# ChenWu98/cycle-diffusion

Measured on AMD Instinct MI355X. Metric: images/sec, SD-v1.4 512px CycleDiffusion 100+100 steps, 1/2/4/8 MI355X, higher is better.
Workload: dtype fp16; 1 GPU; C2: Stable-Diffusion-v1.4-shaped U-Net + KL-f8 VAE, 512x512, custom_steps=99 white_box_steps=100 eta=0.1 skip 0, 1 trial, encoder scale 1, decoder CFG 3; batch_per_gpu=4, global_batch=4, parallelism=dp1, steps_per_launch_set=5, launch_set_cap=16, launch_sets_in_flight_per_gpu=1, images_in_flight_per_gpu=20, distributed=single process, weights=synthetic(seed=0)

## Files before the change

cycle-diffusion_amd/_ffi.py:

```python
import ctypes as C
import os

import numpy as np

_HERE = os.path.dirname(os.path.abspath(__file__))
LIB_PATH = os.path.join(_HERE, "lib", "libcyclediff.so")

CD_NET_UNET_OPENAI, CD_NET_UNET_HO, CD_NET_VAE_KL, CD_NET_CLIP_TEXT, CD_NET_BERT_XTR = 1, 2, 3, 4, 5
CD_NET_OCLIP_TEXT, CD_NET_OCLIP_VISION, CD_NET_INCEPTION_FID, CD_NET_LPIPS = 6, 7, 8, 9
CD_SCHED_DDIM, CD_SCHED_DDPM = 0, 1
CD_PREC_16, CD_PREC_F32, CD_PREC_F32X3 = 0, 1, 2
CD_MASK_QSAMPLE, CD_MASK_ENCODER = 0, 1
MASK_SOURCES = {"q_sample": CD_MASK_QSAMPLE, "encoder": CD_MASK_ENCODER}
ACT_NONE, ACT_SILU, ACT_GELU, ACT_GEGLU, ACT_QGELU, ACT_RELU = 0, 1, 2, 3, 4, 5


class NetDesc(C.Structure):
    _fields_ = [
        ("kind", C.c_int), ("image_size", C.c_int), ("in_channels", C.c_int), ("out_channels", C.c_int),
        ("model_channels", C.c_int), ("num_res_blocks", C.c_int),
        ("n_mult", C.c_int), ("channel_mult", C.c_int * 8),
        ("n_attn", C.c_int), ("attn", C.c_int * 8),
        ("num_heads", C.c_int), ("num_head_channels", C.c_int),
        ("use_spatial_transformer", C.c_int), ("context_dim", C.c_int), ("transformer_depth", C.c_int),
# ... 55 lines not shown
                              _U64, _VP],
    "cd_cycle_translate_masked": [_VP, _I, _I, _VP, _VP, _VP, _F, _VP, _VP, _F, _VP, _I, _I, _I, _I, _VP, _VP, _VP, _U64, _I,
                                  _VP, _VP, _I, _I, _VP, _VP, _U64, _VP, _VP],
    "cd_cycle_translate_ctrl": [_VP, _I, _I, _VP, _VP, _VP, _F, _VP, _VP, _F, _VP, _I, _I, _I, _I, _VP, _VP, _VP, _U64, _I,
                                _VP, _VP, _I, _I, _VP, _VP, _U64, _VP, _VP, _VP, _I, _I, _VP, _VP],
    "cd_cycle_translate_blend": [_VP, _I, _I, _VP, _VP, _VP, _F, _VP, _VP, _F, _VP, _I, _I, _I, _I, _VP, _VP, _VP, _U64, _I,
                                 _VP, _VP, _VP, _I, _I, _VP, _VP, _I, _I, _I, _F, _I, _VP, _VP, _VP, _VP],
    "cd_cycle_translate_sega": [_VP, _I, _I, _VP, _VP, _VP, _F, _VP, _VP, _F, _VP, _I, _I, _I, _I, _VP, _VP, _VP, _U64, _I,
                                _VP, _VP, _I, _I, _VP, _VP, _U64, _VP, _VP, _VP, _I, _I, _VP, _VP, _I, _F, _F, _VP, _VP, _VP,
                                _VP, _VP],
    "cd_ilvr_decode": [_VP, _I, _I, _VP, _I, _I, _I, _I, _VP, _VP, _U64, _VP, _I, _I, _I, _VP, _VP, _U64, _VP],
    "cd_automask": [_VP, _I, _VP, _VP, _VP, _I, _I, _I, _I, _F, _F, _VP, _U64, _I, _F, _F, _I, _VP, _VP],
    "cd_word_maps": [_VP, _I, _VP, _VP, _I, _I, _VP, _I, _I, _I, _I, _F, _F, _VP, _U64, _I, _I, _I, _VP, C.POINTER(_I)],
    "cd_pix_refine": [_VP, _I, _I, _VP, _I, _I, _VP, _VP, _U64],
    "cd_op_pack_conv_weight": [_VP, _VP, _I, _I, _I, _I, _I, C.POINTER(_VP), C.POINTER(_I), C.POINTER(_I)],
    "cd_op_free": [_VP, _VP],
    "cd_op_conv2d": [_VP, _VP, _I, _VP, _I, _I, _I, _I, _VP, _I, _I, _I, _I, _I, _I, _I, _VP, _VP, _VP, _I, _I, _VP],
    "cd_op_conv2d_16": [_VP, _VP, _I, _VP, _I, _I, _I, _I, _VP, _I, _I, _I, _I, _I, _I, _I, _VP, _VP, _VP, _I, _I, _VP,
                        _VP],
    "cd_op_last_gemm_config": [_VP] + [C.POINTER(_I)] * 5,
    "cd_op_up_phase_reorder": [_VP, _VP, _I, _I, _I, _I, _VP],
    "cd_op_groupnorm": [_VP, _VP, _I, _I, _I, _I, _I, _F, _VP, _VP, _VP, _I, _VP],
    "cd_op_groupnorm_ex": [_VP, _VP, _I, _I, _VP, _I, _I, _I, _I, _I, _F, _VP, _VP, _VP, _I, _I, _VP, _VP, _I, _VP],
    "cd_op_pack_conv_weight_prec": [_VP, _VP, _I, _I, _I, _I, _I, C.POINTER(_VP)],
    "cd_op_conv2d_prec": [_VP, _VP, _I, _I, _VP, _I, _I, _I, _I, _I, _VP, _I, _I, _I, _I, _I, _I, _I, _VP, _VP, _I, _VP, _I, _I,
                          _I, _I, _I, _I, _F, _VP, _VP],
    "cd_op_attention_prec": [_VP, _VP, _VP, _VP, _I, _I, _I, _I, _I, _I, _I, _I, _F, _I, _VP, _I, _I, _VP],
    "cd_op_rows_prec": [_VP, _I, _VP, _I64, _I, _I, _VP, _I, _I, _VP, _VP, _I, _VP],
    "cd_op_resample_prec": [_VP, _I, _VP, _I, _I, _I, _I, _I, _VP],
    "cd_op_layernorm": [_VP, _VP, _I, _I, _VP, _VP, _F, _VP],
    "cd_op_st_entry": [_VP, _VP, _I, _I, _I, _VP, _VP, _F, _VP, _VP, _VP, _VP, _VP, _VP, _VP, _I, _VP, _VP, _VP,
                       C.POINTER(_I)],
    "cd_op_attention": [_VP, _VP, _VP, _VP, _I, _I, _I, _I, _I, _F, _I, _VP],
    "cd_op_cross_attention_ctrl": [_VP, _VP, _VP, _VP, _VP, _VP, _VP, _VP, _VP, _I, _I, _I, _I, _I, _I, _I, _I, _F, _VP],
    "cd_op_cross_attention_ctrl_ex": [_VP, _VP, _VP, _VP, _VP, _VP, _VP, _VP, _VP, _I, _I, _I, _I, _I, _I, _I, _I, _F, _I, _I,
                                      _VP],
    "cd_op_cross_attention_maps": [_VP, _VP, _VP, _VP, _I, _I, _I, _I, _I, _I, _I, _I, _F, _I, _VP],
    "cd_op_attention_ex": [_VP, _VP, _VP, _VP, _I, _I, _I, _I, _I, _I, _I, _I, _I, _I, _F, _I, _VP, _I, _I, _VP],
    "cd_op_lowpass": [_VP, _VP, _I, _I, _I, _I, _VP],
    "cd_op_softmax_rows": [_VP, _VP, _I64, _I, _VP],
    "cd_op_timestep_embedding": [_VP, _VP, _I, _I, _I, _VP],
    "cd_op_sched_step": [_VP, _I, _I, _VP, _VP, _VP, _VP, _I, _F, _VP, _VP, _I, _I, _I, _I, _VP],
    "cd_op_gauss": [_VP, _U64, C.c_uint32, _I64, _I64, _VP],
    "cd_op_automask_reduce": [_VP, _VP, _VP, _I, _I, _I, _I, _I, _F, _F, _I, _VP, _VP, _VP],
    "cd_op_local_blend_mask": [_VP, _VP, _VP, _I, _I, _I, _I, _I, _F, _VP],
    "cd_op_sched_step_masked": [_VP, _I, _VP, _VP, _VP, _I, _F, _VP, _VP, _VP, _I, _I, _F, _F, _VP, _I, _I, _I, _I, _VP, _I],
# ... 70 lines not shown
```

cycle-diffusion_amd/build.py:

```python
import os
import subprocess
import sys
from concurrent.futures import ThreadPoolExecutor

HERE = os.path.dirname(os.path.abspath(__file__))
CSRC = os.path.join(HERE, "csrc")
LIBDIR = os.path.join(HERE, "lib")
OBJDIR = os.path.join(HERE, "build")
LIB = os.path.join(LIBDIR, "libcyclediff.so")
SOURCES = ["sched.hip", "sega.hip", "ilvr.hip", "automask.hip", "elementwise.hip", "norm.hip", "conv_gemm.hip", "lin_stream.hip", "attn.hip", "f32_path.hip", "st_f32.hip", "diag.hip", "engine.hip",
           "unet_openai.hip", "nets_ho_vae.hip", "clip_text.hip", "inception.hip", "lpips.hip",
           "capi.hip", "capi_ops.hip"]
HEADERS = ["common.h", "kernels.h", "sched_elem.h", "gauss.h", "engine.h", "capi_internal.h", os.path.join("..", "..", "include", "cyclediff.h")]
FLAGS = ["--offload-arch=gfx950", "-O3", "-std=c++17", "-fPIC", "-Wall", "-Wno-unused-function",
         "-Wno-unused-variable", "-Wno-unused-but-set-variable"]


def _hipcc():
    for cand in (os.environ.get("HIPCC"), "/opt/rocm/bin/hipcc", "hipcc"):
        if cand and (os.path.isabs(cand) and os.path.exists(cand) or not os.path.isabs(cand)):
            return cand
    raise RuntimeError("hipcc not found")


def _stale(target, deps):
    if not os.path.exists(target):
        return True
    t = os.path.getmtime(target)
    return any(os.path.getmtime(d) > t for d in deps)


def build(force=False, verbose=False, variant=None):
    objdir, lib, defines = OBJDIR, LIB, []
    if variant == "bf16":
# ... 41 lines not shown
```

cycle-diffusion_amd/csrc/capi_ops.hip:

```cpp
#include "capi_internal.h"

namespace {

bf16_t* op_rows16(cd_engine* h, const float* src, int64_t rows, int C) {
  bf16_t* d = (bf16_t*)h->arena.alloc((size_t)rows * C * 2);
  launch_nchw_to_nhwc(h->st, src, d, (int)rows, C, 1, C, 1.f, 0.f, 0);
  return d;
}
Act op_image16(Ctx& c, const float* x, int B, int C, int H, int W, int Cpad) {
  Act a = alloc_act(c, B, H, W, Cpad);
  launch_nchw_to_nhwc(c.st, x, a.p, B, C, H * W, Cpad, 1.f, 0.f, 0);
  return a;
}

bf16_t* op_nan_rows16(cd_engine* h, int64_t rows, int ld) {
  const size_t bytes = (size_t)(rows + 64) * ld * 2;
  bf16_t* t = (bf16_t*)h->arena.alloc(bytes);
  HIP_CHECK(hipMemsetAsync(t, 0xFF, bytes, h->st));
  return t;
}
float* op_nan_buffer(cd_engine* h, size_t n) {
  float* t = (float*)h->arena.alloc(n * sizeof(float));
  launch_fill_f32(h->st, t, __builtin_nanf(""), (int64_t)n);
  return t;
// ... 233 lines not shown
  CD_CHECK(h && x0 && gamma && beta && y && B > 0 && H > 0 && W > 0 && C0 > 0 && pad0 >= 0 && pad1 >= 0, "bad argument");
  CD_CHECK(x1 ? C1 > 0 : (C1 == 0 && !stats1), "bad argument (second source)");
  CD_CHECK(precision >= 0 && precision <= 2 && film_ld >= 0, "bad argument (precision 0 = 16-bit, 1 = fp32, 2 = fp32 split)");
  const int align = precision ? 4 : 8;
  CD_CHECK((C0 + pad0) % align == 0 && (C1 + pad1) % align == 0, "row strides must be multiples of %d elements", align);
  ArenaScope arena_scope(h->arena);
  Ctx c = prec_ctx(h, precision);
  const int HW = H * W, C = C0 + C1;
  Act a0 = c.f32 ? op_upload_nhwc(h, x0, B, C0, C0, C0 + pad0, H, W) : op_upload_nhwc16(h, x0, B, C0, C0 + pad0, H, W);
  a0.stats = const_cast<float*>(stats0);
  Act a1;
  if (x1) {
    a1 = c.f32 ? op_upload_nhwc(h, x1, B, C1, C1, C1 + pad1, H, W) : op_upload_nhwc16(h, x1, B, C1, C1 + pad1, H, W);
    a1.stats = const_cast<float*>(stats1);
  }
  GNW w; w.g = const_cast<float*>(gamma); w.b = const_cast<float*>(beta); w.C = C; w.eps = eps;
  Act o = groupnorm_fwd(c, w, a0, x1 ? &a1 : nullptr, silu != 0, film, film_ld);
  if (precision == 2) {
    CD_CHECK(o.split && o.ld == 2 * C, "groupnorm: split output expected");
    op_download(h, o, (size_t)B * HW * C, y);
  } else {
    op_download_nchw(h, o.p, c.f32, o.ld, (float*)y, B, C, HW);
  }
  CD_API_END
}

int cd_op_layernorm(cd_handle h, const float* x, int rows, int C, const float* gamma, const float* beta,
                    float eps, float* y) {
  CD_API_BEGIN
  enter_engine(h);
  CD_CHECK(h && x && y, "bad argument");
  ArenaScope arena_scope(h->arena);
  const bf16_t* a = op_rows16(h, x, rows, C);
  bf16_t* o = (bf16_t*)h->arena.alloc((size_t)rows * C * 2);
  launch_layernorm(h->st, a, C, o, C, rows, C, gamma, beta, eps);
  op_download_nchw(h, o, false, C, y, rows, C, 1);
  CD_API_END
}

int cd_op_st_entry(cd_handle h, const float* x, int B, int H, int W, const float* gn_gamma, const float* gn_beta,
                   float gn_eps, const void* w_in, const float* b_in, const float* ln_gamma, const float* ln_beta,
                   const void* w_qk, const void* w_v, const float* v_bias, int stages, float* h_out, float* qk_out,
                   float* vt_out, int* stages_run) {
  CD_API_BEGIN
  enter_engine(h);
  CD_CHECK(h && x && gn_gamma && gn_beta && w_in && ln_gamma && ln_beta && w_qk && w_v && h_out && qk_out && vt_out &&
// ... 872 lines not shown
```

cycle-diffusion_amd/csrc/kernels.h:

```cpp
#pragma once
#include <map>
#include <string>
#include <vector>

#include "common.h"

namespace cd {

struct StepCoef {
  float sa, s1a, sap, dirc, sigma, r, t_mask;
  int t;
};
enum { SCHED_DDIM = 0, SCHED_DDPM = 1 };

struct EpsHat {
  const float* p = nullptr;
  int64_t sb = 0, sc = 0, sp = 0;
  int cfg = 0;
  float g = 1.f;
  const float* gvec = nullptr;
};

struct StepGeom {
  int B = 0, C = 0, HW = 0;
// ... 224 lines not shown
  const bf16_t* wfrag = nullptr;
  const float* bias = nullptr;
  const bf16_t* resid = nullptr; int ldr = 0;
  bf16_t* out = nullptr; int ldo = 0;
  float* stats = nullptr;
  int M = 0, N = 0;
  float ln_eps = 1e-5f;
  int nsplit = 0, hw = 0;
  bf16_t* vt = nullptr; int vt_ld = 0;
  int64_t vt_bytes = 0;
  const float* gn_coef = nullptr;
};
constexpr int kLinStreamTile = 30;
bool lin_stream_supports(const ConvGemmParams& p);
void launch_lin_stream(hipStream_t st, const ConvGemmParams& p);
bool lin_stream_entry_supports(int64_t M, int hw, int lda);
void launch_lin_stream_qkv(hipStream_t st, const bf16_t* a, int lda, int M, int hw, const bf16_t* wfrag, const float* bias,
                           bf16_t* qk, bf16_t* vt, int vt_ld, bool ln_fold, float ln_eps);
void launch_lin_stream_gn(hipStream_t st, const bf16_t* a, int lda, int M, int hw, const float* gn_coef, const bf16_t* wfrag,
                          const float* bias, bf16_t* out, int ldo);
void launch_fold_ln(hipStream_t st, const bf16_t* w, int ldw, const float* gamma, const float* beta, const float* bias,
                    bf16_t* w_out, float* bias_out, int N, int Kc);
void launch_pack_wfrag(hipStream_t st, const bf16_t* w, int ldw, bf16_t* out, int N);

struct KernelProfiler {
  bool enabled = false;
  std::vector<hipEvent_t> events;
  std::vector<double> flops;
  std::vector<std::string> labels;
  int used = 0;
  bool verbose = false;
  struct Entry { int n = 0; double ms = 0, flops = 0; };
  std::map<std::string, Entry> per_shape;
  void next_pair(hipEvent_t* a, hipEvent_t* b, double fl, const std::string& what);
  void collect(int* launches, double* total_ms, double* total_flops);
  ~KernelProfiler();
};
extern thread_local KernelProfiler* g_conv_prof;

struct ConvTuner {
  bool enabled = false;
  void* scratch = nullptr;
  size_t scratch_bytes = 0;
  int shapes_tuned = 0;
};
extern ConvTuner g_conv_tuner;
// ... 150 lines not shown
```

cycle-diffusion_amd/csrc/unet_openai.hip:

```cpp
#include <algorithm>

#include "engine.h"

namespace cd {

namespace {

struct STW {
  int C = 0, heads = 0, dh = 0, ctx = 0;
  GNW norm;
  ConvW *proj_in = nullptr, *proj_out = nullptr;
  LNW ln1, ln2, ln3;
  ConvW *qkv1 = nullptr, *qk1 = nullptr, *v1 = nullptr, *o1 = nullptr;
  ConvW *q2 = nullptr, *k2 = nullptr, *v2 = nullptr, *o2 = nullptr;
  ConvW *ff1 = nullptr, *ff2 = nullptr;
  ConvW *q2_ln = nullptr, *ff1_ln = nullptr;
  StEntryW entry;
  int side = 0;
  bf16_t* k2c = nullptr;
  bf16_t* v2c = nullptr;
};

struct Layer {
  enum Kind { CONV_IN, RES, ST, AB, DOWN_CONV, UP_CONV } kind;
// ... 3 lines not shown
struct Block { std::vector<Layer> layers; };

class UNetOpenAI : public UNet {
 public:
  explicit UNetOpenAI(const cd_net_desc& d);
  int kind() const override { return CD_NET_UNET_OPENAI; }
  void forward(Ctx& c, const UNetIO& io) override;
  void set_context(Ctx& c, const bf16_t* ctx, int B, int L) override;
  void build_attn_control(Ctx& c, const float* mapper, const float* alpha, const float* weight, int B_ctrl,
                          AttnCtrl& ctrl) override;
  int count_text_blocks(int min_side, int max_side) const override;
  size_t workspace_hint(int B) const override;

 private:
  int mc_, hidden_;
  TimeEmb te_;
  std::vector<ResW> res_;
  std::vector<STW> st_;
  std::vector<AttnW> ab_;
  std::vector<Block> in_blocks_, out_blocks_;
  Block mid_;
  GNW out_norm_;
  ConvW* out_conv_ = nullptr;
  int ctx_B_ = 0, ctx_L_ = 0;
  std::vector<void*> ctx_allocs_;
  const AttnCtrl* ctrl_ = nullptr;
  const WordMapCollect* maps_ = nullptr;

  int add_res(const std::string& pfx, int cin, int cout, bool up, bool down);
  int add_st(const std::string& pfx, int C, int heads, int dh);
  int add_ab(const std::string& pfx, int C, int heads);
  int folded_version_ = -1;
  void refresh_ln_folds(Ctx& c);
  Act run_block(Ctx& c, const Block& b, Act h, const Act* skip, const float* proj, int proj_ld, bool t_shared);
  Act st_fwd(Ctx& c, STW& s, const Act& x, int dup_tail = 0);
  void st_core16(Ctx& c, STW& s, const Act& x_in, const Act& x_resid, Act& out, int dup_tail);
 public:
  ~UNetOpenAI() override { for (void* p : ctx_allocs_) (void)hipFree(p); }
};

int UNetOpenAI::add_res(const std::string& pfx, int cin, int cout, bool up, bool down) {
  ResW r; r.cin = cin; r.cout = cout; r.up = up; r.down = down; r.film = desc.use_scale_shift_norm != 0;
  r.gn1 = make_gn(params, pfx + ".in_layers.0", cin, 1e-5f);
  r.conv1 = make_conv(params, pfx + ".in_layers.2", cout, cin, 3, true);
  r.gn2 = make_gn(params, pfx + ".out_layers.0", cout, 1e-5f);
  r.conv2 = make_conv(params, pfx + ".out_layers.3", cout, cout, 3, true);
// ... 134 lines not shown
    for (int i = 0; i <= d.num_res_blocks; ++i) {
      const int ich = chans.back(); chans.pop_back();
      Block b; Layer l; l.kind = Layer::RES;
      const std::string pfx = "output_blocks." + std::to_string(oi);
      l.idx = add_res_named(pfx + ".0", ch + ich, mc_ * mult, false, false);
      b.layers.push_back(l);
      ch = mc_ * mult;
      int sub = 1;
      if (has_attn(ds)) { add_attn(b, pfx + "." + std::to_string(sub), ch); ++sub; }
      if (level && i == d.num_res_blocks) {
        Layer u;
        const std::string up = pfx + "." + std::to_string(sub);
        if (d.resblock_updown) { u.kind = Layer::RES; u.idx = add_res_named(up, ch, ch, true, false); }
        else { u.kind = Layer::UP_CONV; u.conv = make_conv(params, up + ".conv", ch, ch, 3, true); params.add_up_phase(u.conv); }
        b.layers.push_back(u);
        ds /= 2;
      }
      out_blocks_.push_back(b); ++oi;
    }
  }
  out_norm_ = make_gn(params, "out.0", ch, 1e-5f);
  out_conv_ = make_conv(params, "out.2", d.out_channels, mc_, 3, true);
  CD_CHECK(ch == mc_, "channel bookkeeping: final channels %d != model_channels %d", ch, mc_);

  te_.mode = 0; te_.dim = mc_; te_.hidden = hidden_;
  te_.w0 = params.new_vec(hidden_ * mc_); te_.b0 = params.new_vec(hidden_);
  te_.w1 = params.new_vec(hidden_ * hidden_); te_.b1 = params.new_vec(hidden_);
  params.mat_f32("time_embed.0.weight", te_.w0, hidden_, mc_);
  params.vec("time_embed.0.bias", te_.b0, hidden_);
  params.mat_f32("time_embed.2.weight", te_.w1, hidden_, hidden_);
  params.vec("time_embed.2.bias", te_.b1, hidden_);
  te_.proj_w = params.new_vec(te_.proj_total * hidden_);
  te_.proj_b = params.new_vec(te_.proj_total);
  for (size_t i = 0; i < res_.size(); ++i) {
    const int n = res_[i].film ? 2 * res_[i].cout : res_[i].cout;
    params.mat_f32(res_pfx[i] + ".emb_layers.1.weight", te_.proj_w, n, hidden_, res_[i].emb_off);
    params.bias_rows(res_pfx[i] + ".emb_layers.1.bias", n, te_.proj_b, res_[i].emb_off, n, 0, n, 0);
  }
}

size_t UNetOpenAI::workspace_hint(int B) const {
  const size_t hw = (size_t)image_size * image_size;
  size_t widest = 0;
  for (auto& r : res_) widest = std::max(widest, (size_t)std::max(r.cin, r.cout));
  return (size_t)B * hw * std::max(widest, (size_t)8 * mc_) * 2 * 24 + (64u << 20);
}
// ... 254 lines not shown
    Act g;
    if (s.ff1_ln && conv_ln_fold_available(c, *s.ff1_ln, h.rows())) {
      ConvOpts pl; pl.pad = 0; pl.ln_fold = true;
      g = conv_fwd(c, *s.ff1_ln, h, nullptr, pl);
    } else {
      Act n3 = layernorm_fwd(c, s.ln3, h);
      g = conv_fwd(c, *s.ff1, n3, nullptr, p0);
    }
    ConvOpts o; o.pad = 0; o.resid = &h; o.out = h.p; o.out_ld = h.ld;
    conv_fwd(c, *s.ff2, g, nullptr, o);
    c.arena->release(m2);
  }
  ConvOpts po; po.pad = 0; po.resid = &x; po.out = out.p; po.out_ld = out.ld; po.out_stats = out.stats_buf;
  conv_fwd(c, *s.proj_out, h, nullptr, po);
  c.arena->release(mk);
}

Act UNetOpenAI::run_block(Ctx& c, const Block& b, Act h, const Act* skip, const float* proj, int proj_ld,
                          bool t_shared) {
  bool first = true;
  for (const Layer& l : b.layers) {
    const Act* x2 = first ? skip : nullptr;
    switch (l.kind) {
      case Layer::CONV_IN: { ConvOpts o; o.want_stats = true; h = conv_fwd(c, *l.conv, h, nullptr, o); break; }
      case Layer::RES: h = res_fwd(c, res_[l.idx], h, x2, proj, proj_ld, t_shared); break;
      case Layer::ST: h = st_fwd(c, st_[l.idx], h); break;
      case Layer::AB: h = attn_block_fwd(c, ab_[l.idx], h); break;
      case Layer::DOWN_CONV: { ConvOpts o; o.stride = 2; o.want_stats = true; h = conv_fwd(c, *l.conv, h, nullptr, o); break; }
      case Layer::UP_CONV: { ConvOpts o; o.up = true; o.want_stats = true; h = conv_fwd(c, *l.conv, h, nullptr, o); break; }
    }
    first = false;
  }
  return h;
}

void UNetOpenAI::refresh_ln_folds(Ctx& c) {
  if (folded_version_ == params.version) return;
  for (const Block& b : out_blocks_)
    for (const Layer& l : b.layers)
      if (l.kind == Layer::UP_CONV) params.refresh_up_phase(c.st, l.conv);
  for (STW& s : st_) {
    st_entry_refresh(c.st, s.entry);
    if (!s.q2_ln) continue;
    struct { const ConvW* src; ConvW* dst; const LNW* ln; } jobs[2] = {{s.q2, s.q2_ln, &s.ln2}, {s.ff1, s.ff1_ln, &s.ln3}};
    for (auto& j : jobs) {
      launch_fold_ln(c.st, j.src->w, j.src->Ktot(), j.ln->g, j.ln->b, j.src->b, j.dst->w, j.dst->b, j.src->Npad,
                     j.src->Cpad);
      launch_pack_wfrag(c.st, j.dst->w, j.dst->Ktot(), j.dst->wfrag, j.dst->Npad);
    }
  }
  folded_version_ = params.version;
}

void UNetOpenAI::forward(Ctx& c, const UNetIO& io) {
  const size_t mk0 = c.arena->mark();
  PrecisionScope prec(c, f32, x3);
  refresh_ln_folds(c);
  CD_CHECK(!io.ctrl || (!f32 && io.ctrl->va.size() == st_.size()), "U-Net: cross-attention control on a network it was not built for");
  CD_CHECK(!io.maps || !f32, "U-Net: per-word attention maps are not built for fp32 / fp32x3 networks (their transformer blocks "
           "run the fp32 attention of st_f32.hip): use the 16-bit precision");
  const bool maps_all = io.maps && !io.maps->ranged();
  CD_CHECK(!(maps_all && io.ctrl), "U-Net: a forward collects per-word attention maps or runs cross-attention control, not both");
  CD_CHECK(!maps_all || (io.dup_tail == 0 && !io.cfg_dup), "U-Net: per-word attention maps on a batch with repeated rows");
  ctrl_ = io.ctrl;
  maps_ = io.maps;
  if (maps_) maps_->layers = 0;
  const int B = io.B, R = image_size;
  const float* proj = time_emb_fwd(c, te_, io);
  const int proj_ld = te_.proj_total;
  const Act x = net_input_act(io.xin, B, R, R, in_cpad, f32, x3);
  std::vector<Act> hs;
  Act h = x;
  size_t first_full = 0;
  static const bool cfg_share = [] { const char* e = getenv("CYCLEDIFF_CFG_SHARE"); return !(e && e[0] == '0'); }();
  CD_CHECK(!(io.cfg_dup && io.dup_tail) && io.dup_tail >= 0 && 2 * io.dup_tail <= B, "U-Net: repeated-row description");
  const int dtail = io.cfg_dup ? (B % 2 == 0 ? B / 2 : 0) : io.dup_tail;
  if (dtail > 0 && cfg_share && !f32 && io.t_shared && in_blocks_.size() >= 2 &&
      in_blocks_[0].layers.size() == 1 && in_blocks_[0].layers[0].kind == Layer::CONV_IN &&
      in_blocks_[1].layers.size() == 2 && in_blocks_[1].layers[0].kind == Layer::RES &&
      in_blocks_[1].layers[1].kind == Layer::ST) {
    const int Bh = B - dtail;
    Act xh = x; xh.B = Bh;
    Act h0 = run_block(c, in_blocks_[0], xh, nullptr, proj, proj_ld, true);
    Act h0f = alloc_act(c, B, h0.H, h0.W, h0.C, h0.stats != nullptr);
    CD_CHECK(h0.ld == h0.C, "conv_in output: dense tensor expected");
    const int64_t rows_tail = (int64_t)dtail * h0.H * h0.W;
    dup_rows(c, h0.p, h0f.p, h0.rows(), rows_tail, h0.C);
    if (h0.stats) {
      dup_rows(c, (const bf16_t*)h0.stats, (bf16_t*)h0f.stats_buf, (h0.rows() / 32) * 2, (rows_tail / 32) * 2, h0.C * 2);
      h0f.stats = h0f.stats_buf;
    }
    hs.push_back(h0f);
    const Layer& lr = in_blocks_[1].layers[0];
    const Layer& lt = in_blocks_[1].layers[1];
    Act hr = res_fwd(c, res_[lr.idx], h0, nullptr, proj, proj_ld, true);
    h = st_fwd(c, st_[lt.idx], hr, dtail);
    hs.push_back(h);
    first_full = 2;
  }
  for (size_t bi = first_full; bi < in_blocks_.size(); ++bi) {
    h = run_block(c, in_blocks_[bi], h, nullptr, proj, proj_ld, io.t_shared);
    hs.push_back(h);
  }
  h = run_block(c, mid_, h, nullptr, proj, proj_ld, io.t_shared);
  for (const Block& b : out_blocks_) {
    Act skip = hs.back(); hs.pop_back();
    h = run_block(c, b, h, &skip, proj, proj_ld, io.t_shared);
  }
  Act hn = groupnorm_fwd(c, out_norm_, h, nullptr, true);
  ConvOpts oo; oo.out_f32 = true; oo.out = io.out; oo.out_ld = io.out_ld;
  conv_fwd(c, *out_conv_, hn, nullptr, oo);
  c.arena->release(mk0);
  ctrl_ = nullptr;
  maps_ = nullptr;
}

}

std::unique_ptr<UNet> make_unet_openai(const cd_net_desc& d) { return std::unique_ptr<UNet>(new UNetOpenAI(d)); }

}
```

include/cyclediff.h:

```cpp
#ifndef CYCLEDIFF_H
#define CYCLEDIFF_H
#include <stddef.h>
#include <stdint.h>

#ifdef __cplusplus
extern "C" {
#endif

typedef struct cd_engine* cd_handle;

enum { CD_NET_UNET_OPENAI = 1, CD_NET_UNET_HO = 2, CD_NET_VAE_KL = 3, CD_NET_CLIP_TEXT = 4, CD_NET_BERT_XTR = 5,
       CD_NET_OCLIP_TEXT = 6, CD_NET_OCLIP_VISION = 7, CD_NET_INCEPTION_FID = 8, CD_NET_LPIPS = 9 };
enum { CD_SCHED_DDIM = 0, CD_SCHED_DDPM = 1 };
enum { CD_PREC_16 = 0, CD_PREC_F32 = 1, CD_PREC_F32X3 = 2 };
enum { CD_MASK_QSAMPLE = 0, CD_MASK_ENCODER = 1 };

typedef struct cd_net_desc {
  int kind;
  int image_size;
  int in_channels, out_channels;
  int model_channels;
  int num_res_blocks;
  int n_mult;  int channel_mult[8];
  int n_attn;  int attn[8];
// ... 134 lines not shown
                 int N, int n_draws, int t, float qa, float qb, const float* noise, uint64_t seed, int max_rows,
                 int min_side, int max_side, float* maps_out , int* n_layers_out);

int cd_pix_refine(cd_handle h, int net, int sched_kind, float* x, int B, int R,
                  const cd_step_coef* coef_host, const float* noise, uint64_t seed);

int cd_op_pack_conv_weight(cd_handle h, const float* w_host, int N, int Cin, int KH, int KW, int geglu,
                           void** packed_dev, int* Npad, int* Cpad);
int cd_op_free(cd_handle h, void* dev);
int cd_op_conv2d(cd_handle h, const float* x0, int C0, const float* x1, int C1, int B, int H, int W,
                 const void* packed_w, int N, int KH, int KW, int stride, int pad, int asym_pad, int up,
                 const float* bias, const float* rowvec, const float* resid, int act, int tile, float* y);
int cd_op_conv2d_16(cd_handle h, const float* x0, int C0, const float* x1, int C1, int B, int H, int W,
                    const void* packed_w, int N, int KH, int KW, int stride, int pad, int asym_pad, int up,
                    const float* bias, const float* rowvec, const float* resid, int act, int tile, float* y,
                    float* stats);
int cd_op_last_gemm_config(cd_handle h, int* tile_id, int* bk, int* splitk, int* chm, int* tile_group);
int cd_op_up_phase_reorder(cd_handle h, const float* x, int B, int C, int H, int W, float* y);
int cd_op_groupnorm(cd_handle h, const float* x, int B, int C, int H, int W, int G, float eps,
                    const float* gamma, const float* beta, const float* film, int silu, float* y);
int cd_op_groupnorm_ex(cd_handle h, const float* x0, int C0, int pad0, const float* x1, int C1, int pad1, int B, int H,
                       int W, float eps, const float* gamma, const float* beta, const float* film, int film_ld, int silu,
                       const float* stats0, const float* stats1, int precision, void* y);
int cd_op_pack_conv_weight_prec(cd_handle h, const float* w_host, int N, int Cin, int KH, int KW, int geglu,
                                void** packed_dev);
int cd_op_conv2d_prec(cd_handle h, const float* x0, int C0, int pad0, const float* x1, int C1, int pad1, int B, int H, int W,
                      const void* packed_w, int N, int KH, int KW, int stride, int pad, int asym_pad, int up,
                      const float* bias, const float* rowvec, int rowvec_shared, const float* resid, int resid_pad, int act,
                      int raw_geglu, int tile, int precision, int via_split_rows, float alpha, float* y, float* stats);
int cd_op_attention_prec(cd_handle h, const float* q, const float* k, const float* v, int B, int H, int Tq, int Tk, int D,
                         int padq, int padk, int padv, float scale, int q_log2, const float* obias, int mode, int precision,
                         void* o);
int cd_op_rows_prec(cd_handle h, int op, const float* x0, int64_t rows, int C0, int pad0, const float* x1, int C1, int pad1,
                    const float* gamma, const float* beta, int precision, void* y);
int cd_op_resample_prec(cd_handle h, int op, const float* x, int B, int C, int H, int W, int precision, void* y);
int cd_op_layernorm(cd_handle h, const float* x, int rows, int C, const float* gamma, const float* beta,
                    float eps, float* y);
int cd_op_st_entry(cd_handle h, const float* x, int B, int H, int W, const float* gn_gamma, const float* gn_beta,
                   float gn_eps, const void* w_in, const float* b_in, const float* ln_gamma, const float* ln_beta,
                   const void* w_qk, const void* w_v, const float* v_bias, int stages, float* h_out, float* qk_out,
                   float* vt_out, int* stages_run);
int cd_op_attention(cd_handle h, const float* q, const float* k, const float* v, int B, int H, int Tq,
                    int Tk, int D, float scale, int use_transpose_kernel, float* o);
int cd_op_cross_attention_ctrl(cd_handle h, const float* q_own, const float* q_src, const float* k_own, const float* k_src,
                               const float* v_own, const float* mapper, const float* alpha, const float* weight, int B,
                               int B_src, int B_ctrl, int H, int Tq, int L, int L_buf, int D, float scale, float* o);
// ... 64 lines not shown
```

Before: 3.523 images/s.

## Add specialized U-Net input conv and fused GroupNorm-SiLU-conv output head kernels

Adds two dedicated kernels for the thin ends of the U-Net. One is an input 3x3 conv for at most 8 channels that packs taps into MFMA K-slices, writes the per-tile GroupNorm stats, and duplicates the repeated tail batch in place of separate dup_rows copies. The other is an output head that fuses GroupNorm+SiLU with the 3x3 conv to at most 8 channels, avoiding a materialized normalized tensor and a mostly-padded generic GEMM. Both paths are on by default and can be disabled by environment variables; they add pre-packed weight buffers and new code paths that must match the existing numerics.

```diff
diff --git a/cycle-diffusion_amd/_ffi.py b/cycle-diffusion_amd/_ffi.py
--- a/cycle-diffusion_amd/_ffi.py
+++ b/cycle-diffusion_amd/_ffi.py
@@ -101,6 +101,8 @@
     "cd_op_up_phase_reorder": [_VP, _VP, _I, _I, _I, _I, _VP],
     "cd_op_groupnorm": [_VP, _VP, _I, _I, _I, _I, _I, _F, _VP, _VP, _VP, _I, _VP],
     "cd_op_groupnorm_ex": [_VP, _VP, _I, _I, _VP, _I, _I, _I, _I, _I, _F, _VP, _VP, _VP, _I, _I, _VP, _VP, _I, _VP],
+    "cd_op_out_head": [_VP, _VP, _I, _I, _I, _I, _F, _VP, _VP, _VP, _VP, _I, _I, _VP],
+    "cd_op_in_conv": [_VP, _VP, _I, _I, _I, _I, _I, _VP, _VP, _I, _I, _VP, _VP],
     "cd_op_pack_conv_weight_prec": [_VP, _VP, _I, _I, _I, _I, _I, C.POINTER(_VP)],
     "cd_op_conv2d_prec": [_VP, _VP, _I, _I, _VP, _I, _I, _I, _I, _I, _VP, _I, _I, _I, _I, _I, _I, _I, _VP, _VP, _I, _VP, _I, _I,
                           _I, _I, _I, _I, _F, _VP, _VP],
diff --git a/cycle-diffusion_amd/build.py b/cycle-diffusion_amd/build.py
--- a/cycle-diffusion_amd/build.py
+++ b/cycle-diffusion_amd/build.py
@@ -9,7 +9,7 @@
 OBJDIR = os.path.join(HERE, "build")
 LIB = os.path.join(LIBDIR, "libcyclediff.so")
 SOURCES = ["sched.hip", "sega.hip", "ilvr.hip", "automask.hip", "elementwise.hip", "norm.hip", "conv_gemm.hip", "lin_stream.hip", "attn.hip", "f32_path.hip", "st_f32.hip", "diag.hip", "engine.hip",
-           "unet_openai.hip", "nets_ho_vae.hip", "clip_text.hip", "inception.hip", "lpips.hip",
+           "unet_openai.hip", "unet_ends.hip", "nets_ho_vae.hip", "clip_text.hip", "inception.hip", "lpips.hip",
            "capi.hip", "capi_ops.hip"]
 HEADERS = ["common.h", "kernels.h", "sched_elem.h", "gauss.h", "engine.h", "capi_internal.h", os.path.join("..", "..", "include", "cyclediff.h")]
 FLAGS = ["--offload-arch=gfx950", "-O3", "-std=c++17", "-fPIC", "-Wall", "-Wno-unused-function",
diff --git a/cycle-diffusion_amd/csrc/capi_ops.hip b/cycle-diffusion_amd/csrc/capi_ops.hip
--- a/cycle-diffusion_amd/csrc/capi_ops.hip
+++ b/cycle-diffusion_amd/csrc/capi_ops.hip
@@ -279,6 +279,56 @@
   } else {
     op_download_nchw(h, o.p, c.f32, o.ld, (float*)y, B, C, HW);
   }
+  CD_API_END
+}
+
+int cd_op_out_head(cd_handle h, const float* x, int B, int C, int H, int W, float eps, const float* gamma, const float* beta,
+                   const void* packed_w, const float* bias, int N, int out_ld, float* y) {
+  CD_API_BEGIN
+  enter_engine(h);
+  CD_CHECK(h && x && gamma && beta && packed_w && y && B > 0 && H > 0 && W > 0 && out_ld >= N, "bad argument");
+  const ConvW& w = *(const ConvW*)packed_w;
+  CD_CHECK(w.N == N && w.Cpad == C && out_head_supports(C, N, C, w.KH, w.KW), "out head: 3 x 3, N <= 8, C %% 32 == 0");
+  ArenaScope arena_scope(h->arena);
+  Ctx c = h->ctx();
+  Act a = op_image16(c, x, B, C, H, W, C);
+  GNW g; g.g = const_cast<float*>(gamma); g.b = const_cast<float*>(beta); g.C = C; g.eps = eps;
+  OutHeadParams q;
+  q.x = a.p; q.B = B; q.H = H; q.W = W; q.C = C; q.ld = a.ld;
+  q.coef = groupnorm_coef_fwd(c, g, a);
+  bf16_t* wpk = (bf16_t*)h->arena.alloc((size_t)C * 72 * sizeof(bf16_t));
+  launch_out_head_pack(h->st, w.w, wpk, N, C);
+  q.wpk = wpk; q.bias = bias; q.N = N;
+  const size_t n_out = (size_t)B * H * W * out_ld;
+  q.out = op_nan_buffer(h, n_out); q.out_ld = out_ld;
+  launch_out_head(h->st, q);
+  HIP_CHECK(hipMemcpyAsync(y, q.out, n_out * sizeof(float), hipMemcpyDeviceToDevice, h->st));
+  CD_API_END
+}
+
+int cd_op_in_conv(cd_handle h, const float* x, int B, int C, int in_ld, int H, int W, const void* packed_w, const float* bias,
+                  int N, int dup_tail, float* y, float* stats) {
+  CD_API_BEGIN
+  enter_engine(h);
+  CD_CHECK(h && x && packed_w && y && B > 0 && H > 0 && W > 0 && C > 0 && in_ld >= C && dup_tail >= 0 && dup_tail <= B,
+           "bad argument");
+  const ConvW& w = *(const ConvW*)packed_w;
+  CD_CHECK(w.N == N && w.Cin == C && in_conv_supports(C, N, H, W, in_ld, w.KH, w.KW),
+           "input conv: 3 x 3, C <= 8, N %% 64 == 0, H * W %% 32 == 0, in_ld %% 8 == 0");
+  ArenaScope arena_scope(h->arena);
+  const Act a = op_upload_nhwc16(h, x, B, C, in_ld, H, W);
+  const int Bo = B + dup_tail, HW = H * W;
+  InConvParams q;
+  q.x = a.p; q.B = B; q.H = H; q.W = W; q.C = C; q.ld = in_ld;
+  bf16_t* wpk = (bf16_t*)h->arena.alloc((size_t)5 * N * 16 * sizeof(bf16_t));
+  launch_in_conv_pack(h->st, w.w, wpk, N, w.Cpad);
+  q.wpk = wpk; q.bias = bias; q.N = N; q.dup_tail = dup_tail;
+  q.out = op_nan_rows16(h, (int64_t)Bo * HW, N);
+  const size_t n_stats = (size_t)(Bo * HW / 32) * 2 * N;
+  if (stats) q.stats = op_nan_buffer(h, n_stats);
+  launch_in_conv(h->st, q);
+  op_download_nchw(h, q.out, false, N, y, Bo, N, HW);
+  if (stats) HIP_CHECK(hipMemcpyAsync(stats, q.stats, n_stats * sizeof(float), hipMemcpyDeviceToDevice, h->st));
   CD_API_END
 }
 
diff --git a/cycle-diffusion_amd/csrc/kernels.h b/cycle-diffusion_amd/csrc/kernels.h
--- a/cycle-diffusion_amd/csrc/kernels.h
+++ b/cycle-diffusion_amd/csrc/kernels.h
@@ -270,6 +270,32 @@
 void launch_fold_ln(hipStream_t st, const bf16_t* w, int ldw, const float* gamma, const float* beta, const float* bias,
                     bf16_t* w_out, float* bias_out, int N, int Kc);
 void launch_pack_wfrag(hipStream_t st, const bf16_t* w, int ldw, bf16_t* out, int N);
+
+struct OutHeadParams {
+  const bf16_t* x = nullptr;
+  int B = 0, H = 0, W = 0, C = 0, ld = 0;
+  const float* coef = nullptr;
+  const bf16_t* wpk = nullptr;
+  const float* bias = nullptr;
+  int N = 0;
+  float* out = nullptr; int out_ld = 0;
+};
+bool out_head_supports(int C, int N, int ld, int KH, int KW);
+void launch_out_head_pack(hipStream_t st, const bf16_t* w, bf16_t* wpk, int N, int Cpad);
+void launch_out_head(hipStream_t st, const OutHeadParams& p);
+struct InConvParams {
+  const bf16_t* x = nullptr;
+  int B = 0, H = 0, W = 0, C = 0, ld = 0;
+  const bf16_t* wpk = nullptr;
+  const float* bias = nullptr;
+  int N = 0;
+  bf16_t* out = nullptr;
+  float* stats = nullptr;
+  int dup_tail = 0;
+};
+bool in_conv_supports(int C, int N, int H, int W, int ld, int KH, int KW);
+void launch_in_conv_pack(hipStream_t st, const bf16_t* w, bf16_t* wpk, int N, int Cpad);
+void launch_in_conv(hipStream_t st, const InConvParams& p);
 
 struct KernelProfiler {
   bool enabled = false;
diff --git a/cycle-diffusion_amd/csrc/unet_ends.hip b/cycle-diffusion_amd/csrc/unet_ends.hip
--- /dev/null
+++ b/cycle-diffusion_amd/csrc/unet_ends.hip
@@ -0,0 +1,290 @@
+#include <algorithm>
+
+#include "common.h"
+#include "kernels.h"
+
+namespace cd {
+
+namespace {
+
+constexpr int OH_TW = 32, OH_HW = OH_TW + 2;
+
+template <int NW, int RPW, int KS>
+struct OutHeadGeom {
+  static constexpr int NT = NW * 64, TH = NW * RPW;
+  static constexpr int HP = (TH + 2) * OH_HW;
+  static constexpr int PLANE = HP * 64 + (KS > 1 ? 128 : 0);
+  static constexpr int WSLICE = KS * 9 * 8 * 64;
+  static constexpr int LDS = KS * PLANE + WSLICE;
+  static constexpr int CV = 4 * KS;
+  static constexpr int XV = (HP * CV + NT - 1) / NT;
+  static constexpr int WV = (WSLICE / 16 + NT - 1) / NT;
+};
+
+template <int NW, int RPW, int KS>
+__global__ __launch_bounds__(NW * 64) void k_out_head(OutHeadParams p) {
+  using G = OutHeadGeom<NW, RPW, KS>;
+  __shared__ __attribute__((aligned(16))) unsigned char smem[G::LDS];
+  const int tid = threadIdx.x, lane = tid & 63, wave = tid >> 6;
+  const int tiles_x = (p.W + OH_TW - 1) / OH_TW;
+  const int ty = blockIdx.x / tiles_x, tx = blockIdx.x - ty * tiles_x;
+  const int b = blockIdx.y;
+  const int y0 = ty * G::TH, x0 = tx * OH_TW;
+  const bf16_t* xb = p.x + (int64_t)b * p.H * p.W * p.ld;
+  const float* coef = p.coef + (int64_t)b * 2 * p.C;
+  constexpr int SC = 32 * KS;
+  const int nslice = (p.C + SC - 1) / SC;
+
+  const int cv = tid % G::CV, hp0 = tid / G::CV;
+  int goff[G::XV];
+#pragma unroll
+  for (int i = 0; i < G::XV; ++i) {
+    const int hp = hp0 + (G::NT / G::CV) * i;
+    const int hy = hp / OH_HW, hx = hp - hy * OH_HW;
+    const int y = y0 + hy - 1, x = x0 + hx - 1;
+    goff[i] = (hp < G::HP && y >= 0 && y < p.H && x >= 0 && x < p.W) ? (y * p.W + x) * p.ld : -1;
+  }
+  uint4 xr[G::XV], wr[G::WV];
+  auto issue = [&](int s) __attribute__((always_inline)) {
+    const int c = min(s * SC + cv * 8, p.C - 8);
+#pragma unroll
+    for (int i = 0; i < G::XV; ++i) xr[i] = *(const uint4*)(xb + max(goff[i], 0) + c);
+    const int wvec = min(SC, p.C - s * SC) / 32 * (9 * 8 * 64 / 16);
+#pragma unroll
+    for (int i = 0; i < G::WV; ++i) {
+      const int v = min(tid + G::NT * i, wvec - 1);
+      wr[i] = *(const uint4*)(p.wpk + (int64_t)s * (G::WSLICE / 2) + v * 8);
+    }
+  };
+  auto stage = [&](int s) __attribute__((always_inline)) {
+    const bool cok = s * SC + cv * 8 < p.C;
+    const int c = min(s * SC + cv * 8, p.C - 8);
+    float ca[8], cb[8];
+    {
+      const f32x4 a0 = *(const f32x4*)(coef + c), a1 = *(const f32x4*)(coef + c + 4);
+      const f32x4 b0 = *(const f32x4*)(coef + p.C + c), b1 = *(const f32x4*)(coef + p.C + c + 4);
+#pragma unroll
+      for (int e = 0; e < 4; ++e) { ca[e] = a0[e]; ca[4 + e] = a1[e]; cb[e] = b0[e]; cb[4 + e] = b1[e]; }
+    }
+    unsigned char* plane = smem + (cv >> 2) * G::PLANE + (cv & 3) * 16;
+#pragma unroll
+    for (int i = 0; i < G::XV; ++i) {
+      const int hp = hp0 + (G::NT / G::CV) * i;
+      if (hp < G::HP) {
+        float f[8];
+        unpack8(xr[i], f);
+#pragma unroll
+        for (int e = 0; e < 8; ++e) f[e] = silu_f(f[e] * ca[e] + cb[e]);
+        uint4 o = pack8(f);
+        const unsigned keep = (goff[i] >= 0 && cok) ? 0xffffffffu : 0u;
+        o.x &= keep; o.y &= keep; o.z &= keep; o.w &= keep;
+        *(uint4*)(plane + hp * 64) = o;
+      }
+    }
+#pragma unroll
+    for (int i = 0; i < G::WV; ++i) {
+      const int v = tid + G::NT * i;
+      if (v < G::WSLICE / 16) *(uint4*)(smem + KS * G::PLANE + v * 16) = wr[i];
+    }
+  };
+
+  f32x4 acc[RPW][2];
+#pragma unroll
+  for (int r = 0; r < RPW; ++r)
+#pragma unroll
+    for (int h = 0; h < 2; ++h) acc[r][h] = (f32x4){0.f, 0.f, 0.f, 0.f};
+  const int fp = lane & 15, fk = lane >> 4;
+
+  issue(0);
+  for (int s = 0; s < nslice; ++s) {
+    stage(s);
+    __syncthreads();
+    if (s + 1 < nslice) issue(s + 1);
+    const int ksteps = min(SC, p.C - s * SC) / 32;
+#pragma unroll
+    for (int ks = 0; ks < KS; ++ks) {
+      if (ks < ksteps) {
+        const unsigned char* ap = smem + ks * G::PLANE + fk * 16;
+        const unsigned char* wp = smem + KS * G::PLANE + ks * (9 * 8 * 64) + (fp & 7) * 64 + fk * 16;
+        bf16x8 bw[9];
+#pragma unroll
+        for (int t = 0; t < 9; ++t) bw[t] = *(const bf16x8*)(wp + t * (8 * 64));
+#pragma unroll
+        for (int rr = 0; rr < RPW + 2; ++rr)
+#pragma unroll
+          for (int dx = 0; dx < 3; ++dx)
+#pragma unroll
+            for (int h = 0; h < 2; ++h) {
+              const int hp = (RPW * wave + rr) * OH_HW + 16 * h + dx + fp;
+              const bf16x8 a = *(const bf16x8*)(ap + hp * 64);
+#pragma unroll
+              for (int dy = 0; dy < 3; ++dy) {
+                const int r = rr - dy;
+                if (r >= 0 && r < RPW) acc[r][h] = CD_MFMA_16x16x32(a, bw[dy * 3 + dx], acc[r][h]);
+              }
+            }
+      }
+    }
+    __syncthreads();
+  }
+
+  if (fp < p.N) {
+    const float bias = p.bias ? p.bias[fp] : 0.f;
+#pragma unroll
+    for (int r = 0; r < RPW; ++r)
+#pragma unroll
+      for (int h = 0; h < 2; ++h)
+#pragma unroll
+        for (int e = 0; e < 4; ++e) {
+          const int y = y0 + RPW * wave + r, x = x0 + 16 * h + 4 * fk + e;
+          if (y < p.H && x < p.W) p.out[((int64_t)(b * p.H + y) * p.W + x) * p.out_ld + fp] = acc[r][h][e] + bias;
+        }
+  }
+}
+
+__global__ __launch_bounds__(256) void k_out_head_pack(const bf16_t* __restrict__ w, bf16_t* __restrict__ out, int N, int Cpad) {
+  const int total = (Cpad / 32) * 9 * 8 * 32;
+  for (int i = blockIdx.x * 256 + threadIdx.x; i < total; i += gridDim.x * 256) {
+    const int c = i & 31, n = (i >> 5) & 7, t = (i >> 8) % 9, kc = (i >> 8) / 9;
+    out[i] = n < N ? w[(int64_t)n * 9 * Cpad + t * Cpad + kc * 32 + c] : (bf16_t)0;
+  }
+}
+
+constexpr int IC_ELD = 144;
+
+__global__ __launch_bounds__(256) void k_in_conv(InConvParams p) {
+  __shared__ __attribute__((aligned(16))) unsigned char smem[4 * 32 * IC_ELD];
+  const int lane = threadIdx.x & 63, wave = threadIdx.x >> 6;
+  const int nchunk = p.N >> 6;
+  const int chunk = blockIdx.x % nchunk, grp = blockIdx.x / nchunk, ngrp = gridDim.x / nchunk;
+  const int fr = lane & 31, fh = lane >> 5;
+  const int n0 = chunk * 64;
+  unsigned char* E = smem + wave * 32 * IC_ELD;
+
+  bf16x8 bw[5][2];
+#pragma unroll
+  for (int s = 0; s < 5; ++s)
+#pragma unroll
+    for (int j = 0; j < 2; ++j)
+      bw[s][j] = *(const bf16x8*)(p.wpk + ((int64_t)(s * p.N + n0 + j * 32 + fr) * 16 + fh * 8));
+  const float bias0 = p.bias ? p.bias[n0 + fr] : 0.f, bias1 = p.bias ? p.bias[n0 + 32 + fr] : 0.f;
+  uint4 cmask;
+  {
+    unsigned m[4];
+#pragma unroll
+    for (int i = 0; i < 4; ++i) m[i] = (2 * i + 1 < p.C ? 0xffff0000u : 0u) | (2 * i < p.C ? 0x0000ffffu : 0u);
+    cmask = make_uint4(m[0], m[1], m[2], m[3]);
+  }
+  const int HW = p.H * p.W;
+  const int nblk = p.B * (HW >> 5);
+  const int dup_blk0 = (p.B - p.dup_tail) * (HW >> 5);
+  const int dup_shift = p.dup_tail * (HW >> 5);
+
+  for (int blk = grp * 4 + wave; blk < nblk; blk += ngrp * 4) {
+    const int m = blk * 32 + fr;
+    const int b = m / HW, pix = m - b * HW;
+    const int y = pix / p.W, x = pix - y * p.W;
+    uint4 a[5];
+#pragma unroll
+    for (int s = 0; s < 5; ++s) {
+      const int t = 2 * s + fh;
+      const int dy = t / 3 - 1, dx = t - (t / 3) * 3 - 1;
+      const int yy = y + dy, xx = x + dx;
+      const bool ok = t < 9 && yy >= 0 && yy < p.H && xx >= 0 && xx < p.W;
+      const int src = ok ? (b * p.H + yy) * p.W + xx : m;
+      const uint4 v = *(const uint4*)(p.x + (int64_t)src * p.ld);
+      const unsigned keep = ok ? 0xffffffffu : 0u;
+      a[s] = make_uint4(v.x & cmask.x & keep, v.y & cmask.y & keep, v.z & cmask.z & keep, v.w & cmask.w & keep);
+    }
+    f32x16 acc[2];
+#pragma unroll
+    for (int j = 0; j < 2; ++j) {
+#pragma unroll
+      for (int r = 0; r < 16; ++r) acc[j][r] = 0.f;
+#pragma unroll
+      for (int s = 0; s < 5; ++s) acc[j] = CD_MFMA_32x32x16(__builtin_bit_cast(bf16x8, a[s]), bw[s][j], acc[j]);
+    }
+    __builtin_amdgcn_wave_barrier();
+#pragma unroll
+    for (int j = 0; j < 2; ++j) {
+      const float bias = j ? bias1 : bias0;
+      float sum = 0.f, sq = 0.f;
+#pragma unroll
+      for (int r = 0; r < 16; ++r) {
+        const float v = acc[j][r] + bias;
+        sum += v; sq += v * v;
+        const int row = (r & 3) + 8 * (r >> 2) + 4 * fh;
+        *(bf16_t*)(E + row * IC_ELD + (j * 32 + fr) * 2) = (bf16_t)(pack2(v, 0.f) & 0xffffu);
+      }
+      const float osum = __shfl_xor(sum, 32), osq = __shfl_xor(sq, 32);
+      const float tot = fh ? sq + osq : sum + osum;
+      if (p.stats) {
+        float* sp = p.stats + ((int64_t)blk * 2 + fh) * p.N + n0 + j * 32 + fr;
+        *sp = tot;
+        if (blk >= dup_blk0) sp[(int64_t)dup_shift * 2 * p.N] = tot;
+      }
+    }
+    __builtin_amdgcn_wave_barrier();
+    const int vr = lane >> 3, vc = lane & 7;
+#pragma unroll
+    for (int ps = 0; ps < 4; ++ps) {
+      const int row = ps * 8 + vr;
+      const uint4 o = *(const uint4*)(E + row * IC_ELD + vc * 16);
+      bf16_t* op = p.out + ((int64_t)blk * 32 + row) * p.N + n0 + vc * 8;
+      *(uint4*)op = o;
+      if (blk >= dup_blk0) *(uint4*)(op + (int64_t)dup_shift * 32 * p.N) = o;
+    }
+    __builtin_amdgcn_wave_barrier();
+  }
+}
+
+__global__ __launch_bounds__(256) void k_in_conv_pack(const bf16_t* __restrict__ w, bf16_t* __restrict__ out, int N, int Cpad) {
+  const int total = 5 * N * 16;
+  for (int i = blockIdx.x * 256 + threadIdx.x; i < total; i += gridDim.x * 256) {
+    const int kk = i & 15, n = (i >> 4) % N, s = (i >> 4) / N;
+    const int t = 2 * s + (kk >> 3), c = kk & 7;
+    out[i] = t < 9 ? w[(int64_t)n * 9 * Cpad + t * Cpad + c] : (bf16_t)0;
+  }
+}
+
+}
+
+bool out_head_supports(int C, int N, int ld, int KH, int KW) {
+  return KH == 3 && KW == 3 && N >= 1 && N <= 8 && C > 0 && C % 32 == 0 && ld == C;
+}
+
+void launch_out_head_pack(hipStream_t st, const bf16_t* w, bf16_t* wpk, int N, int Cpad) {
+  CD_CHECK(w && wpk && N >= 1 && N <= 8 && Cpad % 32 == 0, "out head: weight packing");
+  hipLaunchKernelGGL(k_out_head_pack, dim3(ceil_div(Cpad * 72, 256)), dim3(256), 0, st, w, wpk, N, Cpad);
+}
+
+void launch_out_head(hipStream_t st, const OutHeadParams& p) {
+  CD_CHECK(p.x && p.coef && p.wpk && p.out && p.B > 0 && p.H > 0 && p.W > 0, "out head: bad argument");
+  CD_CHECK(out_head_supports(p.C, p.N, p.ld, 3, 3) && p.out_ld >= p.N, "out head: C=%d N=%d ld=%d unsupported", p.C, p.N, p.ld);
+  CD_CHECK((int64_t)p.B * p.H * p.W * p.ld < (1ll << 31) && p.B <= 65535, "out head: tensor too large");
+  constexpr int NW = 8, RPW = 2;
+  hipLaunchKernelGGL((k_out_head<NW, RPW, 1>), dim3(ceil_div(p.H, NW * RPW) * ceil_div(p.W, OH_TW), p.B), dim3(NW * 64), 0, st, p);
+}
+
+bool in_conv_supports(int C, int N, int H, int W, int ld, int KH, int KW) {
+  return KH == 3 && KW == 3 && C >= 1 && C <= 8 && N > 0 && N % 64 == 0 && (H * W) % 32 == 0 && ld >= 8 && ld % 8 == 0;
+}
+
+void launch_in_conv_pack(hipStream_t st, const bf16_t* w, bf16_t* wpk, int N, int Cpad) {
+  CD_CHECK(w && wpk && N > 0 && Cpad >= 8, "input conv: weight packing");
+  hipLaunchKernelGGL(k_in_conv_pack, dim3(ceil_div(5 * N * 16, 256)), dim3(256), 0, st, w, wpk, N, Cpad);
+}
+
+void launch_in_conv(hipStream_t st, const InConvParams& p) {
+  CD_CHECK(p.x && p.wpk && p.out && p.B > 0, "input conv: bad argument");
+  CD_CHECK(in_conv_supports(p.C, p.N, p.H, p.W, p.ld, 3, 3), "input conv: C=%d N=%d %dx%d ld=%d unsupported", p.C, p.N, p.H, p.W,
+           p.ld);
+  CD_CHECK(p.dup_tail >= 0 && p.dup_tail <= p.B, "input conv: repeated tail of %d images in a batch of %d", p.dup_tail, p.B);
+  CD_CHECK((int64_t)(p.B + p.dup_tail) * p.H * p.W < (1ll << 31) / 32, "input conv: tensor too large");
+  const int nchunk = p.N / 64;
+  const int nblk = p.B * (p.H * p.W / 32);
+  const int ngrp = std::max(1, std::min(ceil_div(nblk, 4), 768 / nchunk));
+  hipLaunchKernelGGL(k_in_conv, dim3(ngrp * nchunk), dim3(256), 0, st, p);
+}
+
+}
diff --git a/cycle-diffusion_amd/csrc/unet_openai.hip b/cycle-diffusion_amd/csrc/unet_openai.hip
--- a/cycle-diffusion_amd/csrc/unet_openai.hip
+++ b/cycle-diffusion_amd/csrc/unet_openai.hip
@@ -49,6 +49,9 @@
   Block mid_;
   GNW out_norm_;
   ConvW* out_conv_ = nullptr;
+  ConvW *out_head_w_ = nullptr, *in_conv_w_ = nullptr;
+  bool in_conv_taken(const Ctx& c, const ConvW& w, const Act& x) const;
+  Act in_conv_fwd(Ctx& c, const ConvW& w, const Act& x, int dup_tail);
   int ctx_B_ = 0, ctx_L_ = 0;
   std::vector<void*> ctx_allocs_;
   const AttnCtrl* ctrl_ = nullptr;
@@ -229,6 +232,10 @@
   out_norm_ = make_gn(params, "out.0", ch, 1e-5f);
   out_conv_ = make_conv(params, "out.2", d.out_channels, mc_, 3, true);
   CD_CHECK(ch == mc_, "channel bookkeeping: final channels %d != model_channels %d", ch, mc_);
+  if (!f32) {
+    if (out_head_supports(mc_, d.out_channels, mc_, 3, 3)) out_head_w_ = params.new_conv(8, mc_, 3, 3, false);
+    if (d.in_channels <= 8 && mc_ % 64 == 0) in_conv_w_ = params.new_conv(mc_, 8, 3, 3, false);
+  }
 
   te_.mode = 0; te_.dim = mc_; te_.hidden = hidden_;
   te_.w0 = params.new_vec(hidden_ * mc_); te_.b0 = params.new_vec(hidden_);
@@ -529,7 +536,10 @@
   for (const Layer& l : b.layers) {
     const Act* x2 = first ? skip : nullptr;
     switch (l.kind) {
-      case Layer::CONV_IN: { ConvOpts o; o.want_stats = true; h = conv_fwd(c, *l.conv, h, nullptr, o); break; }
+      case Layer::CONV_IN: {
+        if (in_conv_taken(c, *l.conv, h)) { h = in_conv_fwd(c, *l.conv, h, 0); break; }
+        ConvOpts o; o.want_stats = true; h = conv_fwd(c, *l.conv, h, nullptr, o); break;
+      }
       case Layer::RES: h = res_fwd(c, res_[l.idx], h, x2, proj, proj_ld, t_shared); break;
       case Layer::ST: h = st_fwd(c, st_[l.idx], h); break;
       case Layer::AB: h = attn_block_fwd(c, ab_[l.idx], h); break;
@@ -543,6 +553,11 @@
 
 void UNetOpenAI::refresh_ln_folds(Ctx& c) {
   if (folded_version_ == params.version) return;
+  if (out_head_w_) launch_out_head_pack(c.st, out_conv_->w, out_head_w_->w, out_conv_->N, out_conv_->Cpad);
+  if (in_conv_w_) {
+    const ConvW* ci = in_blocks_[0].layers[0].conv;
+    launch_in_conv_pack(c.st, ci->w, in_conv_w_->w, ci->N, ci->Cpad);
+  }
   for (const Block& b : out_blocks_)
     for (const Layer& l : b.layers)
       if (l.kind == Layer::UP_CONV) params.refresh_up_phase(c.st, l.conv);
@@ -557,6 +572,23 @@
     }
   }
   folded_version_ = params.version;
+}
+
+bool UNetOpenAI::in_conv_taken(const Ctx& c, const ConvW& w, const Act& x) const {
+  static const bool on = [] { const char* e = getenv("CYCLEDIFF_IN_CONV"); return !(e && e[0] == '0'); }();
+  return on && in_conv_w_ && !c.f32 && !x.f32 && !x.split && w.Cpad <= x.ld &&
+         in_conv_supports(desc.in_channels, w.N, x.H, x.W, x.ld, w.KH, w.KW);
+}
+
+Act UNetOpenAI::in_conv_fwd(Ctx& c, const ConvW& w, const Act& x, int dup_tail) {
+  Act y = alloc_act(c, x.B + dup_tail, x.H, x.W, w.N, true);
+  InConvParams q;
+  q.x = x.p; q.B = x.B; q.H = x.H; q.W = x.W; q.C = desc.in_channels; q.ld = x.ld;
+  q.wpk = in_conv_w_->w; q.bias = w.b; q.N = w.N;
+  q.out = y.p; q.stats = y.stats_buf; q.dup_tail = dup_tail;
+  launch_in_conv(c.st, q);
+  y.stats = y.stats_buf;
+  return y;
 }
 
 void UNetOpenAI::forward(Ctx& c, const UNetIO& io) {
@@ -588,14 +620,21 @@
       in_blocks_[1].layers[1].kind == Layer::ST) {
     const int Bh = B - dtail;
     Act xh = x; xh.B = Bh;
-    Act h0 = run_block(c, in_blocks_[0], xh, nullptr, proj, proj_ld, true);
-    Act h0f = alloc_act(c, B, h0.H, h0.W, h0.C, h0.stats != nullptr);
-    CD_CHECK(h0.ld == h0.C, "conv_in output: dense tensor expected");
-    const int64_t rows_tail = (int64_t)dtail * h0.H * h0.W;
-    dup_rows(c, h0.p, h0f.p, h0.rows(), rows_tail, h0.C);
-    if (h0.stats) {
-      dup_rows(c, (const bf16_t*)h0.stats, (bf16_t*)h0f.stats_buf, (h0.rows() / 32) * 2, (rows_tail / 32) * 2, h0.C * 2);
-      h0f.stats = h0f.stats_buf;
+    Act h0, h0f;
+    const ConvW& cin = *in_blocks_[0].layers[0].conv;
+    if (in_conv_taken(c, cin, xh)) {
+      h0f = in_conv_fwd(c, cin, xh, dtail);
+      h0 = h0f; h0.B = Bh;
+    } else {
+      h0 = run_block(c, in_blocks_[0], xh, nullptr, proj, proj_ld, true);
+      h0f = alloc_act(c, B, h0.H, h0.W, h0.C, h0.stats != nullptr);
+      CD_CHECK(h0.ld == h0.C, "conv_in output: dense tensor expected");
+      const int64_t rows_tail = (int64_t)dtail * h0.H * h0.W;
+      dup_rows(c, h0.p, h0f.p, h0.rows(), rows_tail, h0.C);
+      if (h0.stats) {
+        dup_rows(c, (const bf16_t*)h0.stats, (bf16_t*)h0f.stats_buf, (h0.rows() / 32) * 2, (rows_tail / 32) * 2, h0.C * 2);
+        h0f.stats = h0f.stats_buf;
+      }
     }
     hs.push_back(h0f);
     const Layer& lr = in_blocks_[1].layers[0];
@@ -614,9 +653,20 @@
     Act skip = hs.back(); hs.pop_back();
     h = run_block(c, b, h, &skip, proj, proj_ld, io.t_shared);
   }
-  Act hn = groupnorm_fwd(c, out_norm_, h, nullptr, true);
-  ConvOpts oo; oo.out_f32 = true; oo.out = io.out; oo.out_ld = io.out_ld;
-  conv_fwd(c, *out_conv_, hn, nullptr, oo);
+  static const bool out_head_on = [] { const char* e = getenv("CYCLEDIFF_OUT_HEAD"); return !(e && e[0] == '0'); }();
+  if (out_head_on && out_head_w_ && !f32 && !h.split && h.C == out_conv_->Cpad && io.out_ld >= out_conv_->N &&
+      out_head_supports(h.C, out_conv_->N, h.ld, out_conv_->KH, out_conv_->KW)) {
+    OutHeadParams q;
+    q.x = h.p; q.B = h.B; q.H = h.H; q.W = h.W; q.C = h.C; q.ld = h.ld;
+    q.coef = groupnorm_coef_fwd(c, out_norm_, h);
+    q.wpk = out_head_w_->w; q.bias = out_conv_->b; q.N = out_conv_->N;
+    q.out = io.out; q.out_ld = io.out_ld;
+    launch_out_head(c.st, q);
+  } else {
+    Act hn = groupnorm_fwd(c, out_norm_, h, nullptr, true);
+    ConvOpts oo; oo.out_f32 = true; oo.out = io.out; oo.out_ld = io.out_ld;
+    conv_fwd(c, *out_conv_, hn, nullptr, oo);
+  }
   c.arena->release(mk0);
   ctrl_ = nullptr;
   maps_ = nullptr;
diff --git a/include/cyclediff.h b/include/cyclediff.h
--- a/include/cyclediff.h
+++ b/include/cyclediff.h
@@ -180,6 +180,10 @@
 int cd_op_groupnorm_ex(cd_handle h, const float* x0, int C0, int pad0, const float* x1, int C1, int pad1, int B, int H,
                        int W, float eps, const float* gamma, const float* beta, const float* film, int film_ld, int silu,
                        const float* stats0, const float* stats1, int precision, void* y);
+int cd_op_out_head(cd_handle h, const float* x, int B, int C, int H, int W, float eps, const float* gamma, const float* beta,
+                   const void* packed_w, const float* bias, int N, int out_ld, float* y);
+int cd_op_in_conv(cd_handle h, const float* x, int B, int C, int in_ld, int H, int W, const void* packed_w, const float* bias,
+                  int N, int dup_tail, float* y, float* stats);
 int cd_op_pack_conv_weight_prec(cd_handle h, const float* w_host, int N, int Cin, int KH, int KW, int geglu,
                                 void** packed_dev);
 int cd_op_conv2d_prec(cd_handle h, const float* x0, int C0, int pad0, const float* x1, int C1, int pad1, int B, int H, int W,
```

Result: no change. 3.539 images/s, median of 6 (+0.4%).
